# EnricoMiccoli/nodal

Measured on NVIDIA B200. Metric: unknowns_per_second, higher is better.
Workload: dtype f64

## Files before the change

__graft_entry__.py:

```python
import os
import subprocess
import sys

ROOT = os.path.dirname(os.path.abspath(__file__))
if ROOT not in sys.path:
    sys.path.insert(0, ROOT)


def build():
    subprocess.check_call(["make", "-C", os.path.join(ROOT, "nodal_b200", "csrc"), "-j8"])
    sys.path.insert(0, os.path.join(ROOT, "tests"))
    import helpers
    helpers.stamp_host_lib()
    helpers.amg_host_lib()
    import sources_host
    sources_host.sources_host_lib()
    import amg_cycle_host
    amg_cycle_host.amg_cycle_host_lib()
    ref_nodal = os.path.join(os.environ.get("NODAL_REFERENCE", "/root/reference"), "nodal")
    if os.path.isdir(ref_nodal) and not os.path.isfile(os.path.join(ROOT, "baseline", "_ref", "nodal", "nodal.py")):
        subprocess.call([sys.executable, os.path.join(ROOT, "baseline", "install_ref.py")])
    import nodal_b200
    from nodal_b200 import _lib
    _lib.load()


def smoke():
    import numpy as np
    import nodal_b200 as n
    import nodal_b200.equiv
    from nodal_b200 import dist as ndist
    from nodal_b200 import generators as gen
    from nodal_b200.device import Device
    from oracle import mna_oracle as orc

    N = 24
    r_cpu = orc.equivalent_resistance(orc.grid2d_rows(N), "1", "g", sparse=True, backend="dict")
    r_gpu = n.equiv.equivalent_resistance(gen.grid2d(N), "1", "g", sparse=True)
    r_jac = n.equiv.equivalent_resistance(gen.grid2d(N), "1", "g", sparse=True, precond="jacobi")
    r_amg = n.equiv.equivalent_resistance(gen.grid2d(N), "1", "g", sparse=True, precond="amg", amg={"coarse": 64})
    for r in (r_gpu, r_jac, r_amg):
        assert abs(r - r_cpu) <= 1e-9 * abs(r_cpu), (r, r_cpu)
    dev = Device.get(0)
    import copy
    net = copy.deepcopy(gen.grid2d(64))
    net.process_component(["a1", "A", "1", "1", "g"])
    table = net.table()
    csr, rhs = dev.assemble_csr(table)
    x, info = ndist.single_solver(dev).solve_amg(csr.n, np.array([0, csr.n], dtype=np.int32), csr.indptr, csr.indices,
                                                  csr.data, rhs, rtol=1e-10, gather_below=300)
    r_dist = float(x[net.nodenum["1"]])
    r64 = orc.equivalent_resistance(orc.grid2d_rows(64), "1", "g", sparse=True, backend="dict")
    assert info["status"] == 0 and info["distributed_levels"] >= 1 and abs(r_dist - r64) <= 1e-9 * abs(r64), (info, r_dist, r64)
    pg = gen.power_grid(16, 5, vdd=1.0, load=1e-3, seed=0)
    sol = n.Circuit(pg, sparse=True, eliminate_sources=True).solve()
    red = sol.stats["reduction"]
    assert red["eliminated"] and red["relres_full"] <= 1e-9 and np.all(sol.potentials() <= 1.0), sol.stats
    print(f"smoke ok: R({N}x{N} grid) default={float(r_gpu)!r} jacobi={float(r_jac)!r} amg={float(r_amg)!r} "
          f"oracle={float(r_cpu)!r}; R(64x64) partitioned-AMG form={r_dist!r} oracle={float(r64)!r}; "
          f"power grid 16x16 relres_full={red['relres_full']:.1e}")


if __name__ == "__main__":
    build()
    if len(sys.argv) > 1 and sys.argv[1] == "smoke":
        smoke()
```

include/nodal_b200.h:

```cpp
#ifndef NODAL_B200_H
#define NODAL_B200_H

#include <stdint.h>

#ifdef __cplusplus
extern "C" {
#endif

#define NODAL_ABI_VERSION 1

enum {
    NODAL_OK = 0,
    NODAL_SINGULAR = 1,
    NODAL_NOT_CONVERGED = 2,
    NODAL_BREAKDOWN = 3,
    NODAL_CUDA_ERROR = 4,
    NODAL_BAD_ARG = -1
};

enum { NODAL_T_R = 0, NODAL_T_A = 1, NODAL_T_E = 2, NODAL_T_VCVS = 3, NODAL_T_VCCS = 4,
       NODAL_T_CCVS = 5, NODAL_T_CCCS = 6 };
#define NODAL_GROUND (-1)
#define NODAL_UNUSED (-2)

typedef struct nodal_ctx nodal_ctx;

int nodal_abi_version(void);
const char* nodal_last_error(void);
uint64_t nodal_launch_count(void);
int nodal_ctx_create(int device, nodal_ctx** out);
int nodal_ctx_destroy(nodal_ctx* ctx);
int64_t nodal_ctx_workspace_bytes(nodal_ctx* ctx);

int nodal_stamp_coo(nodal_ctx* ctx, int64_t ncomp,
                    const uint8_t* type, const double* value,
                    const int32_t* a, const int32_t* b, const int32_t* c, const int32_t* d,
                    const int32_t* drv, const int32_t* branch,
                    int32_t kcl, int32_t n, int32_t stride, int32_t colbits,
                    uint64_t* keys, double* vals, void* stream);

int nodal_csr_build(nodal_ctx* ctx, int32_t n, int64_t nslots, int32_t colbits,
                    uint64_t* keys, double* vals, double* rhs,
                    int64_t* nnz_h, void* stream);
int nodal_csr_fetch(nodal_ctx* ctx, int32_t n, int64_t nnz,
                    int32_t* indptr, int32_t* indices, double* data, void* stream);
int nodal_csr_build_ordered(nodal_ctx* ctx, int32_t n, int64_t nslots, int32_t colbits,
                            uint64_t* keys, double* vals, int32_t order, double* rhs, int64_t* nnz_h,
                            void* stream);

int nodal_csr_to_dense(nodal_ctx* ctx, int32_t n, const int32_t* indptr, const int32_t* indices,
                       const double* data, double* G, void* stream);
int nodal_coo_to_dense_atomic(nodal_ctx* ctx, int32_t n, int64_t nslots, int32_t colbits,
                              const uint64_t* keys, const double* vals, double* G, double* rhs,
                              void* stream);

int nodal_spmv(nodal_ctx* ctx, int32_t n, int64_t nnz, const int32_t* indptr,
               const int32_t* indices, const double* data, const double* x, double* y,
               void* stream);

typedef struct nodal_sell nodal_sell;
int nodal_sell_create(nodal_ctx* ctx, int32_t n, int64_t nnz, const int32_t* indptr,
                      const int32_t* indices, const double* data, nodal_sell** out, void* stream);
int nodal_sell_destroy(nodal_sell* m);
int64_t nodal_sell_padded_nnz(const nodal_sell* m);
int nodal_sell_spmv(nodal_ctx* ctx, const nodal_sell* m, const double* x, double* y, void* stream);

int nodal_pcg(nodal_ctx* ctx, int32_t n, int64_t nnz, const int32_t* indptr,
              const int32_t* indices, const double* data, const double* rhs, double* x,
              double rtol, int32_t maxit, int32_t flags,
              int32_t* iters_h, double* relres_h, double* stats_h, void* stream);
#define NODAL_PCG_FORCE_CSR 1
#define NODAL_PCG_NO_GRAPH 2
#define NODAL_PCG_PROFILE 4
#define NODAL_PCG_NO_SCALE 8

int nodal_gmres(nodal_ctx* ctx, int32_t n, int64_t nnz, const int32_t* indptr,
                const int32_t* indices, const double* data, const double* rhs, double* x,
                double rtol, int32_t restart, int32_t maxit,
                int32_t* iters_h, double* relres_h, void* stream);

typedef struct nodal_amg nodal_amg;
int nodal_amg_create(nodal_ctx* ctx, int32_t n, int64_t nnz, const int32_t* indptr,
                     const int32_t* indices, const double* data, const double* params,
                     nodal_amg** out, void* stream);
int nodal_amg_destroy(nodal_amg* amg);
int nodal_amg_info(const nodal_amg* amg, int32_t cap, int32_t* nlevels, int64_t* rows, int64_t* nnz,
                   double* setup_ms, int32_t* direct);
int nodal_amg_fetch_level(nodal_ctx* ctx, const nodal_amg* amg, int32_t level, int32_t* agg,
                          int32_t* indptr, int32_t* indices, double* data, void* stream);
int nodal_amg_apply(nodal_ctx* ctx, const nodal_amg* amg, const double* r, double* z, void* stream);
int nodal_amg_pcg(nodal_ctx* ctx, nodal_amg* amg, const double* rhs, double* x, double rtol,
                  int32_t maxit, int32_t* iters_h, double* relres_h, double* stats_h, void* stream);

int nodal_connected_components(nodal_ctx* ctx, int64_t ncomp, const int32_t* a, const int32_t* b,
                               int32_t kcl, int32_t* labels, int32_t* ncomponents_h,
                               int32_t* reached_h, void* stream);

int nodal_source_forest(nodal_ctx* ctx, int64_t ncomp, const uint8_t* type, const double* value,
                        const int32_t* a, const int32_t* b, const int32_t* branch, int32_t kcl, int32_t be,
                        int32_t* erow, int32_t* adj_ptr, int32_t* adj_row, int32_t* rep_row, double* offset,
                        int32_t* parent_edge, int32_t* depth, int32_t* roots, int64_t* info_h, void* stream);
int nodal_source_reduce_scan(nodal_ctx* ctx, int64_t ncomp, const uint8_t* type, const int32_t* a,
                             const int32_t* b, int32_t kcl, const int32_t* rep_row, const double* offset,
                             uint32_t* pos, int64_t* count_h, void* stream);
int nodal_source_reduce_table(nodal_ctx* ctx, int64_t ncomp, const uint8_t* type, const double* value,
                              const int32_t* a, const int32_t* b, int32_t kcl, const int32_t* rep_row,
                              const double* offset, const uint32_t* pos, uint8_t* out_type, double* out_value,
                              int32_t* out_a, int32_t* out_b, void* stream);
int nodal_source_expand(nodal_ctx* ctx, int32_t kcl, int32_t n, int32_t nsrc, const int32_t* erow,
                        const int32_t* a, const int32_t* b, const int32_t* branch, const int32_t* adj_ptr,
                        const int32_t* adj_row, const int32_t* rep_row, const double* offset,
                        const int32_t* depth, int32_t max_depth, const double* y, const double* rhs,
                        int64_t nnz, const int32_t* indptr, const int32_t* indices, const double* data,
                        double* x, double* relres_h, void* stream);

int nodal_lu_solve(nodal_ctx* ctx, int32_t n, double* G, const double* rhs, double* x,
                   int32_t* info_h, void* stream);

int nodal_dgemm_sub_profile(nodal_ctx* ctx, double* C, const double* A, const double* B, int32_t M, int32_t N,
                            int32_t K, int32_t ld, int32_t reps, double* ms_out, void* stream);

int nodal_lu_batched(nodal_ctx* ctx, int64_t batch, int32_t ncomp,
                     const uint8_t* type, const int32_t* a, const int32_t* b,
                     const int32_t* c, const int32_t* d, const int32_t* drv, const int32_t* branch,
                     int32_t kcl, int32_t n, const double* values, double* x, int32_t* info,
                     void* stream);

int nodal_lu_batched_soa(nodal_ctx* ctx, int64_t batch, int32_t ncomp,
                         const uint8_t* type, const int32_t* a, const int32_t* b,
                         const int32_t* c, const int32_t* d, const int32_t* drv, const int32_t* branch,
                         int32_t kcl, int32_t n, const double* values_t, double* x_t, int32_t* info,
// ... 41 lines not shown
```

nodal_b200/_lib.py:

```python
from __future__ import annotations

import ctypes as C
import os

_HERE = os.path.dirname(os.path.abspath(__file__))
LIB_PATH = os.path.join(_HERE, "libnodal_b200.so")

OK, SINGULAR, NOT_CONVERGED, BREAKDOWN, CUDA_ERROR, BAD_ARG = 0, 1, 2, 3, 4, -1
PCG_FORCE_CSR, PCG_NO_GRAPH, PCG_PROFILE, PCG_NO_SCALE = 1, 2, 4, 8

_vp, _i32, _i64, _f64 = C.c_void_p, C.c_int32, C.c_int64, C.c_double

SIGNATURES = {
    "nodal_abi_version": (C.c_int, []),
    "nodal_last_error": (C.c_char_p, []),
    "nodal_launch_count": (C.c_uint64, []),
    "nodal_ctx_create": (C.c_int, [C.c_int, C.POINTER(_vp)]),
    "nodal_ctx_destroy": (C.c_int, [_vp]),
    "nodal_ctx_workspace_bytes": (_i64, [_vp]),
    "nodal_stamp_coo": (C.c_int, [_vp, _i64, _vp, _vp, _vp, _vp, _vp, _vp, _vp, _vp,
                                  _i32, _i32, _i32, _i32, _vp, _vp, _vp]),
    "nodal_csr_build": (C.c_int, [_vp, _i32, _i64, _i32, _vp, _vp, _vp, C.POINTER(_i64), _vp]),
    "nodal_csr_build_ordered": (C.c_int, [_vp, _i32, _i64, _i32, _vp, _vp, _i32, _vp, C.POINTER(_i64), _vp]),
    "nodal_csr_fetch": (C.c_int, [_vp, _i32, _i64, _vp, _vp, _vp, _vp]),
    "nodal_csr_to_dense": (C.c_int, [_vp, _i32, _vp, _vp, _vp, _vp, _vp]),
    "nodal_coo_to_dense_atomic": (C.c_int, [_vp, _i32, _i64, _i32, _vp, _vp, _vp, _vp, _vp]),
    "nodal_spmv": (C.c_int, [_vp, _i32, _i64, _vp, _vp, _vp, _vp, _vp, _vp]),
    "nodal_sell_create": (C.c_int, [_vp, _i32, _i64, _vp, _vp, _vp, C.POINTER(_vp), _vp]),
    "nodal_sell_destroy": (C.c_int, [_vp]),
    "nodal_sell_padded_nnz": (_i64, [_vp]),
    "nodal_sell_spmv": (C.c_int, [_vp, _vp, _vp, _vp, _vp]),
    "nodal_pcg": (C.c_int, [_vp, _i32, _i64, _vp, _vp, _vp, _vp, _vp, _f64, _i32, _i32,
                            C.POINTER(_i32), C.POINTER(_f64), C.POINTER(_f64), _vp]),
    "nodal_gmres": (C.c_int, [_vp, _i32, _i64, _vp, _vp, _vp, _vp, _vp, _f64, _i32, _i32,
                              C.POINTER(_i32), C.POINTER(_f64), _vp]),
    "nodal_amg_create": (C.c_int, [_vp, _i32, _i64, _vp, _vp, _vp, C.POINTER(_f64), C.POINTER(_vp), _vp]),
    "nodal_amg_destroy": (C.c_int, [_vp]),
    "nodal_amg_info": (C.c_int, [_vp, _i32, C.POINTER(_i32), C.POINTER(_i64), C.POINTER(_i64),
                                 C.POINTER(_f64), C.POINTER(_i32)]),
    "nodal_amg_fetch_level": (C.c_int, [_vp, _vp, _i32, _vp, _vp, _vp, _vp, _vp]),
    "nodal_amg_apply": (C.c_int, [_vp, _vp, _vp, _vp, _vp]),
    "nodal_amg_pcg": (C.c_int, [_vp, _vp, _vp, _vp, _f64, _i32, C.POINTER(_i32), C.POINTER(_f64),
                                C.POINTER(_f64), _vp]),
    "nodal_connected_components": (C.c_int, [_vp, _i64, _vp, _vp, _i32, _vp, C.POINTER(_i32),
                                             C.POINTER(_i32), _vp]),
    "nodal_source_forest": (C.c_int, [_vp, _i64, _vp, _vp, _vp, _vp, _vp, _i32, _i32] + [_vp] * 8
                            + [C.POINTER(_i64), _vp]),
    "nodal_source_reduce_scan": (C.c_int, [_vp, _i64, _vp, _vp, _vp, _i32, _vp, _vp, _vp, C.POINTER(_i64), _vp]),
    "nodal_source_reduce_table": (C.c_int, [_vp, _i64, _vp, _vp, _vp, _vp, _i32, _vp, _vp, _vp, _vp, _vp, _vp, _vp,
                                            _vp]),
    "nodal_source_expand": (C.c_int, [_vp, _i32, _i32, _i32] + [_vp] * 9 + [_i32, _vp, _vp, _i64, _vp, _vp, _vp, _vp,
                                                                             C.POINTER(_f64), _vp]),
    "nodal_lu_solve": (C.c_int, [_vp, _i32, _vp, _vp, _vp, C.POINTER(_i32), _vp]),
    "nodal_dgemm_sub_profile": (C.c_int, [_vp, _vp, _vp, _vp, _i32, _i32, _i32, _i32, _i32, C.POINTER(_f64), _vp]),
    "nodal_lu_batched": (C.c_int, [_vp, _i64, _i32, _vp, _vp, _vp, _vp, _vp, _vp, _vp,
                                   _i32, _i32, _vp, _vp, _vp, _vp]),
    "nodal_lu_batched_soa": (C.c_int, [_vp, _i64, _i32, _vp, _vp, _vp, _vp, _vp, _vp, _vp,
                                       _i32, _i32, _vp, _vp, _vp, _vp]),
    "nodal_dist_unique_id": (C.c_int, [_vp]),
    "nodal_dist_create": (C.c_int, [_vp, _vp, _i32, _i32, C.POINTER(_vp)]),
    "nodal_dist_create_single": (C.c_int, [_vp, C.POINTER(_vp)]),
    "nodal_dist_destroy": (C.c_int, [_vp]),
    "nodal_dist_pcg": (C.c_int, [_vp, _vp, _i32, _vp, _i64, _vp, _vp, _vp, _vp, _vp, _f64, _i32,
                                 C.POINTER(_i32), C.POINTER(_f64), C.POINTER(_f64), _vp]),
    "nodal_amg_pcg_multi": (C.c_int, [_vp, _vp, _i32, _vp, _vp, _f64, _i32, C.POINTER(_i32), C.POINTER(_f64),
                                      C.POINTER(_i32), _vp]),
    "nodal_amg_profile_sweeps": (C.c_int, [_vp, _vp, _i32, C.POINTER(_f64), _vp]),
    "nodal_amg_profile_cycle": (C.c_int, [_vp, _vp, _i32, C.POINTER(_f64), _vp]),
    "nodal_table_select_scan": (C.c_int, [_vp, _i64, _vp, _vp, _i32, _i32, _vp, C.POINTER(_i64), _vp]),
    "nodal_table_select_gather": (C.c_int, [_vp, _i64, _vp, _i32, _i32] + [_vp] * 16 + [_vp]),
    "nodal_dist_amg_pcg": (C.c_int, [_vp, _vp, _i32, _vp, _i64, _vp, _vp, _vp, _vp, _vp, C.POINTER(_f64), _f64,
                                     _i32, C.POINTER(_i32), C.POINTER(_f64), C.POINTER(_f64), _vp]),
}

_lib = None


class NodalLibraryError(RuntimeError):
    """The CUDA extension is missing or a CUDA call failed."""


def load():
    global _lib
    if _lib is not None:
        return _lib
    if not os.path.exists(LIB_PATH):
        raise NodalLibraryError(
            f"{LIB_PATH} not found: build it with `python -c 'import __graft_entry__ as g; g.build()'`"
            " (or `make -C nodal_b200/csrc`). nodal_b200 has no CPU fallback.")
    lib = C.CDLL(LIB_PATH)
    for name, (res, args) in SIGNATURES.items():
        fn = getattr(lib, name)
        fn.restype = res
        fn.argtypes = args
    if lib.nodal_abi_version() != 1:
        raise NodalLibraryError("libnodal_b200.so ABI version mismatch")
    _lib = lib
    return lib


def last_error():
    return load().nodal_last_error().decode("utf-8", "replace")


def check(status, what, allowed=(OK,)):
    if status in allowed:
        return status
# ... 2 lines not shown
```

nodal_b200/csrc/common.cuh:

```cuda
#pragma once
#include <cuda_runtime.h>
#include <stdint.h>
#include <stdio.h>
#include <string.h>
#include <string>
#include <vector>

#include "../../include/nodal_b200.h"

#include <nvtx3/nvToolsExt.h>

struct NvtxRange {
    explicit NvtxRange(const char* name) { nvtxRangePushA(name); }
    ~NvtxRange() { nvtxRangePop(); }
    NvtxRange(const NvtxRange&) = delete;
    NvtxRange& operator=(const NvtxRange&) = delete;
};

typedef unsigned long long u64;
typedef unsigned int u32;

#define NODAL_NUM_SMS_FALLBACK 148

void nodal_set_error(const char* fmt, ...);

#define CUDA_TRY(expr)                                                                   \
    do {                                                                                 \
        cudaError_t _e = (expr);                                                         \
        if (_e != cudaSuccess) {                                                         \
            nodal_set_error("%s:%d: %s -> %s", __FILE__, __LINE__, #expr,                \
                            cudaGetErrorString(_e));                                     \
            (void)cudaGetLastError();                       \
            return NODAL_CUDA_ERROR;                                                     \
        }                                                                                \
    } while (0)

#define NODAL_TRY(expr)                                                                  \
    do {                                                                                 \
        int _s = (expr);                                                                 \
        if (_s != NODAL_OK) return _s;                                                   \
    } while (0)

extern unsigned long long g_nodal_launches;
#define KERNEL_CHECK()                 \
    do {                               \
        ++g_nodal_launches;            \
        CUDA_TRY(cudaGetLastError());  \
    } while (0)

struct nodal_ctx {
    int device = 0;
    int num_sms = NODAL_NUM_SMS_FALLBACK;
    char* arena = nullptr;
    size_t arena_bytes = 0;
    size_t arena_used = 0;
    uint64_t generation = 0;
    void* pinned = nullptr;
    struct PoolBlock { void* ptr; size_t bytes; bool used; };
    std::vector<PoolBlock> pool;
};

void* ctx_pool_alloc(nodal_ctx* ctx, size_t bytes);
void ctx_pool_free(nodal_ctx* ctx, void* ptr);

int ctx_reserve(nodal_ctx* ctx, size_t bytes);
void* ctx_carve(nodal_ctx* ctx, size_t bytes);

template <typename T>
static inline T* carve(nodal_ctx* ctx, size_t count) {
    return reinterpret_cast<T*>(ctx_carve(ctx, count * sizeof(T)));
}
static inline size_t align_up(size_t x, size_t a) { return (x + a - 1) / a * a; }

#ifdef __CUDACC__
__device__ __forceinline__ double warp_sum(double v) {
#pragma unroll
    for (int o = 16; o > 0; o >>= 1) v += __shfl_xor_sync(0xffffffffu, v, o);
    return v;
}
__device__ __forceinline__ u32 lane_id() { return threadIdx.x & 31; }
__device__ __forceinline__ u32 lanemask_lt() {
    u32 m;
    asm("mov.u32 %0, %%lanemask_lt;" : "=r"(m));
    return m;
}

__device__ __forceinline__ double block_sum(double v, double* smem ) {
    v = warp_sum(v);
    const int w = threadIdx.x >> 5, nw = (blockDim.x + 31) >> 5;
    __syncthreads();
    if (lane_id() == 0) smem[w] = v;
    __syncthreads();
    if (w == 0) {
        double t = (lane_id() < nw) ? smem[lane_id()] : 0.0;
        t = warp_sum(t);
        if (lane_id() == 0) smem[32] = t;
    }
    __syncthreads();
    return smem[32];
}

__device__ __forceinline__ double reduce_partials(const double* __restrict__ part, int count,
                                                  double* smem) {
    double t = 0.0;
    for (int i = threadIdx.x; i < count; i += blockDim.x) t += part[i];
    return block_sum(t, smem);
}

__device__ __forceinline__ void reduce_partials3(const double* __restrict__ a, int na,
                                                 const double* __restrict__ b, int nb,
                                                 const double* __restrict__ c, int nc, double* smem,
                                                 double& sa, double& sb, double& sc) {
    double va[8], vb[8], vc[8];
#pragma unroll
    for (int k = 0; k < 8; ++k) {
        const int i = threadIdx.x + k * blockDim.x;
        va[k] = i < na ? a[i] : 0.0;
        vb[k] = i < nb ? b[i] : 0.0;
        vc[k] = i < nc ? c[i] : 0.0;
    }
    double ta = 0.0, tb = 0.0, tc = 0.0;
#pragma unroll
    for (int k = 0; k < 8; ++k) {
        const int i = threadIdx.x + k * blockDim.x;
        if (i < na) ta += va[k];
        if (i < nb) tb += vb[k];
        if (i < nc) tc += vc[k];
    }
    sa = block_sum(ta, smem);
    sb = nb > 0 ? block_sum(tb, smem) : 0.0;
    sc = nc > 0 ? block_sum(tc, smem) : 0.0;
}
#endif

int scan_exclusive_u32(nodal_ctx* ctx, const u32* in, u32* out, int64_t count, u32* total_dev,
                       cudaStream_t st);
size_t scan_scratch_bytes(int64_t count);
int radix_sort_pairs(nodal_ctx* ctx, u64* keys, u64* vals, u64* keys_alt, u64* vals_alt,
                     int64_t count, int bits, bool* result_in_alt, cudaStream_t st);
size_t radix_sort_scratch_bytes(int64_t count);
// ... 4 lines not shown
```

nodal_b200/csrc/csr.cu:

```cuda
#include "common.cuh"

constexpr int CB_THREADS = 256;

__global__ void __launch_bounds__(CB_THREADS)
mark_heads_kernel(const u64* __restrict__ keys, int64_t count, int32_t n, int colbits,
                  u32* __restrict__ head) {
    for (int64_t i = (int64_t)blockIdx.x * blockDim.x + threadIdx.x; i < count;
         i += (int64_t)gridDim.x * blockDim.x) {
        const u64 k = keys[i];
        const bool live = (int64_t)(k >> colbits) < (int64_t)n;
        head[i] = (live && (i == 0 || keys[i - 1] != k)) ? 1u : 0u;
    }
}

__global__ void __launch_bounds__(CB_THREADS)
segment_sum_kernel(const u64* __restrict__ keys, const double* __restrict__ vals, int64_t count,
                   int32_t n, int colbits, const u32* __restrict__ head_scan,
                   u64* __restrict__ ukey, double* __restrict__ uval, u32* __restrict__ keep,
                   double* __restrict__ rhs) {
    const u64 colmask = ((u64)1 << colbits) - 1;
    for (int64_t i = (int64_t)blockIdx.x * blockDim.x + threadIdx.x; i < count;
         i += (int64_t)gridDim.x * blockDim.x) {
        const u64 k = keys[i];
        if ((int64_t)(k >> colbits) >= (int64_t)n) continue;
        if (i != 0 && keys[i - 1] == k) continue;
        double s = vals[i];
        for (int64_t j = i + 1; j < count && keys[j] == k; ++j) s = s + vals[j];
        const u32 seg = head_scan[i];
        const int32_t col = (int32_t)(k & colmask);
        ukey[seg] = k;
        uval[seg] = s;
        if (col == n) {
            rhs[(int32_t)(k >> colbits)] = s;
            keep[seg] = 0u;
        } else {
            keep[seg] = (s != 0.0) ? 1u : 0u;
        }
    }
}

__global__ void __launch_bounds__(CB_THREADS)
iota_u64_kernel(int64_t count, u64* __restrict__ out) {
    for (int64_t i = (int64_t)blockIdx.x * blockDim.x + threadIdx.x; i < count; i += (int64_t)gridDim.x * blockDim.x)
        out[i] = (u64)i;
}

__global__ void __launch_bounds__(CB_THREADS)
segment_sum_first_touch_kernel(const u64* __restrict__ keys, const u64* __restrict__ idx, const double* __restrict__ vals,
                               int64_t count, int32_t n, int colbits, const u32* __restrict__ head_scan,
                               u64* __restrict__ ukey, double* __restrict__ uval, u32* __restrict__ keep,
                               u32* __restrict__ ufirst, double* __restrict__ rhs) {
    const u64 colmask = ((u64)1 << colbits) - 1;
    for (int64_t i = (int64_t)blockIdx.x * blockDim.x + threadIdx.x; i < count;
         i += (int64_t)gridDim.x * blockDim.x) {
        const u64 k = keys[i];
        if ((int64_t)(k >> colbits) >= (int64_t)n) continue;
        if (i != 0 && keys[i - 1] == k) continue;
        double s = 0.0;
        bool absent = true;
        u32 first = 0;
        for (int64_t j = i; j < count && keys[j] == k; ++j) {
            const double t = s + vals[idx[j]];
            if (t != 0.0) {
                if (absent) { first = (u32)idx[j]; absent = false; }
            } else {
                absent = true;
            }
            s = absent ? 0.0 : t;
        }
        const u32 seg = head_scan[i];
        const int32_t col = (int32_t)(k & colmask);
        ukey[seg] = k;
        uval[seg] = s;
        ufirst[seg] = first;
        if (col == n) {
            rhs[(int32_t)(k >> colbits)] = s;
            keep[seg] = 0u;
        } else {
            keep[seg] = absent ? 0u : 1u;
        }
    }
}

// ... 2 lines not shown
                        const u32* __restrict__ keep, int64_t useg, int colbits, u64* __restrict__ keys2,
                        u64* __restrict__ pos2) {
    for (int64_t s = (int64_t)blockIdx.x * blockDim.x + threadIdx.x; s < useg; s += (int64_t)gridDim.x * blockDim.x) {
        if (!keep[s]) continue;
        const u32 p = keep_scan[s];
        keys2[p] = ((ukey[s] >> colbits) << 32) | (u64)ufirst[s];
        pos2[p] = (u64)p;
    }
}

__global__ void __launch_bounds__(CB_THREADS)
permute_entries_kernel(int64_t nnz, const u64* __restrict__ pos, const int32_t* __restrict__ cols_in,
                       const double* __restrict__ vals_in, int32_t* __restrict__ cols_out, double* __restrict__ vals_out) {
    for (int64_t q = (int64_t)blockIdx.x * blockDim.x + threadIdx.x; q < nnz; q += (int64_t)gridDim.x * blockDim.x) {
        const u64 p = pos[q];
        cols_out[q] = cols_in[p];
        vals_out[q] = vals_in[p];
    }
}

__global__ void __launch_bounds__(CB_THREADS)
compact_kernel(const u64* __restrict__ ukey, const double* __restrict__ uval,
               const u32* __restrict__ keep_scan, const u32* __restrict__ keep_flag_src,
               int64_t useg, int colbits, int32_t* __restrict__ indices, double* __restrict__ data,
               int32_t* __restrict__ krow) {
    const u64 colmask = ((u64)1 << colbits) - 1;
    for (int64_t s = (int64_t)blockIdx.x * blockDim.x + threadIdx.x; s < useg;
         s += (int64_t)gridDim.x * blockDim.x) {
        if (!keep_flag_src[s]) continue;
        const u32 p = keep_scan[s];
        const u64 k = ukey[s];
        indices[p] = (int32_t)(k & colmask);
        data[p] = uval[s];
        krow[p] = (int32_t)(k >> colbits);
    }
}

struct RowGap { int32_t first, last, value; int32_t pad; };
constexpr int ROWPTR_INLINE = 32;
constexpr int ROWPTR_MAX_GAPS = 4096;

__device__ __forceinline__ void fill_rows(int32_t first, int32_t last, int32_t value,
                                          int32_t* __restrict__ indptr, RowGap* gaps, unsigned int* ngaps) {
    if (last - first < ROWPTR_INLINE) {
        for (int32_t q = first; q <= last; ++q) indptr[q] = value;
        return;
    }
    const unsigned int slot = atomicAdd(ngaps, 1u);
    if (slot < ROWPTR_MAX_GAPS) { gaps[slot].first = first; gaps[slot].last = last; gaps[slot].value = value; }
    else for (int32_t q = first; q <= last; ++q) indptr[q] = value;
}

__global__ void __launch_bounds__(CB_THREADS)
row_ptr_kernel(const int32_t* __restrict__ krow, int64_t nnz, int32_t n,
               int32_t* __restrict__ indptr, RowGap* gaps, unsigned int* ngaps) {
    for (int64_t p = (int64_t)blockIdx.x * blockDim.x + threadIdx.x; p < nnz;
         p += (int64_t)gridDim.x * blockDim.x) {
        const int32_t r = krow[p];
        const int32_t rp = p ? krow[p - 1] : -1;
        if (r != rp) fill_rows(rp + 1, r, (int32_t)p, indptr, gaps, ngaps);
        if (p == nnz - 1) fill_rows(r + 1, n, (int32_t)nnz, indptr, gaps, ngaps);
    }
}

__global__ void __launch_bounds__(CB_THREADS)
row_ptr_gaps_kernel(int32_t* __restrict__ indptr, const RowGap* __restrict__ gaps,
                    const unsigned int* __restrict__ ngaps) {
    const unsigned int count = min(*ngaps, (unsigned int)ROWPTR_MAX_GAPS);
    for (unsigned int g = 0; g < count; ++g) {
        const RowGap gp = gaps[g];
        for (int64_t q = (int64_t)gp.first + (int64_t)blockIdx.x * blockDim.x + threadIdx.x; q <= gp.last;
             q += (int64_t)gridDim.x * blockDim.x)
            indptr[q] = gp.value;
    }
}

static int grid_for(nodal_ctx* ctx, int64_t work, int threads) {
    int64_t b = (work + threads - 1) / threads;
    int64_t cap = (int64_t)ctx->num_sms * 16;
    if (b < 1) b = 1;
    return (int)(b < cap ? b : cap);
}

struct PendingCsr {
    nodal_ctx* ctx = nullptr;
    const u64* ukey = nullptr;
    const double* uval = nullptr;
    const u32* keep = nullptr;
    const u32* keep_scan = nullptr;
    int32_t* krow = nullptr;
    const u32* ufirst = nullptr;
    int order = 0;
    int64_t useg = 0, nnz = 0;
    int32_t n = 0;
    int colbits = 0;
    uint64_t generation = 0;
};
static thread_local PendingCsr g_pending;

static int csr_build_impl(nodal_ctx* ctx, int32_t n, int64_t nslots, int32_t colbits, uint64_t* keys_, double* vals,
                          double* rhs, int64_t* nnz_h, void* stream, int order);

extern "C" int nodal_csr_build(nodal_ctx* ctx, int32_t n, int64_t nslots, int32_t colbits,
                               uint64_t* keys_, double* vals, double* rhs, int64_t* nnz_h,
                               void* stream) {
    return csr_build_impl(ctx, n, nslots, colbits, keys_, vals, rhs, nnz_h, stream, 0);
}

extern "C" int nodal_csr_build_ordered(nodal_ctx* ctx, int32_t n, int64_t nslots, int32_t colbits,
                                       uint64_t* keys_, double* vals, int32_t order, double* rhs,
                                       int64_t* nnz_h, void* stream) {
    if (order != 0 && order != 1) return NODAL_BAD_ARG;
    return csr_build_impl(ctx, n, nslots, colbits, keys_, vals, rhs, nnz_h, stream, order);
}

static int csr_build_impl(nodal_ctx* ctx, int32_t n, int64_t nslots, int32_t colbits, uint64_t* keys_, double* vals,
                          double* rhs, int64_t* nnz_h, void* stream, int order) {
    NvtxRange nvtx_range("nodal_csr_build");
    if (!ctx || n < 0 || nslots < 0 || !nnz_h) return NODAL_BAD_ARG;
    if (nslots >= ((int64_t)1 << 31)) {
        nodal_set_error("nodal_csr_build: more than 2^31 triples are not supported");
        return NODAL_BAD_ARG;
    }
    cudaStream_t st = (cudaStream_t)stream;
    u64* keys = reinterpret_cast<u64*>(keys_);
    g_pending = PendingCsr();
    *nnz_h = 0;
    CUDA_TRY(cudaSetDevice(ctx->device));
    CUDA_TRY(cudaMemsetAsync(rhs, 0, sizeof(double) * (size_t)n, st));
    if (nslots == 0 || n == 0) {
        g_pending.ctx = ctx;
        g_pending.n = n;
        NODAL_TRY(ctx_reserve(ctx, 4096));
        g_pending.generation = ctx->generation;
        return NODAL_OK;
    }
    int rowbits = 1;
    while (((int64_t)n >> rowbits) != 0) ++rowbits;
    const int bits = colbits + rowbits;

    const size_t slots = (size_t)nslots;
    size_t need = 2 * align_up(slots * 8, 256) + 3 * align_up(slots * 4, 256) +
                  radix_sort_scratch_bytes(nslots) + 2 * scan_scratch_bytes(nslots) + (1 << 16);
    if (order == 1) need += 2 * align_up(slots * 8, 256) + align_up(slots * 4, 256);
    NODAL_TRY(ctx_reserve(ctx, need));
    u64* keys_alt = carve<u64>(ctx, slots);
    u64* vals_alt = carve<u64>(ctx, slots);
    u64* idx = order == 1 ? carve<u64>(ctx, slots) : nullptr;
    double* usum = order == 1 ? carve<double>(ctx, slots) : nullptr;
    u32* ufirst = order == 1 ? carve<u32>(ctx, slots) : nullptr;
    if (order == 1 && (!idx || !usum || !ufirst)) return NODAL_CUDA_ERROR;
    u32* head = carve<u32>(ctx, slots);
    u32* keep = carve<u32>(ctx, slots);
    u32* keep_scan = carve<u32>(ctx, slots);
    u32* totals = carve<u32>(ctx, 64);
    if (!keys_alt || !vals_alt || !head || !keep || !keep_scan || !totals) return NODAL_CUDA_ERROR;

    bool in_alt = false;
    const size_t mark = ctx->arena_used;
    const int grid = grid_for(ctx, nslots, CB_THREADS);
    if (order == 1) {
        iota_u64_kernel<<<grid, CB_THREADS, 0, st>>>(nslots, idx);
        KERNEL_CHECK();
    }
    NODAL_TRY(radix_sort_pairs(ctx, keys, order == 1 ? idx : reinterpret_cast<u64*>(vals), keys_alt, vals_alt, nslots,
                               bits, &in_alt, st));
    ctx->arena_used = mark;
    const u64* sk = in_alt ? keys_alt : keys;
    const double* sv = in_alt ? reinterpret_cast<double*>(vals_alt) : vals;
    const u64* sidx = in_alt ? vals_alt : idx;
    u64* ukey = in_alt ? keys : keys_alt;
    double* uval = order == 1 ? usum : (in_alt ? vals : reinterpret_cast<double*>(vals_alt));

    mark_heads_kernel<<<grid, CB_THREADS, 0, st>>>(sk, nslots, n, colbits, head);
    KERNEL_CHECK();
    NODAL_TRY(scan_exclusive_u32(ctx, head, head, nslots, totals + 0, st));
    ctx->arena_used = mark;
    if (order == 1)
        segment_sum_first_touch_kernel<<<grid, CB_THREADS, 0, st>>>(sk, sidx, vals, nslots, n, colbits, head, ukey, uval,
                                                                    keep, ufirst, rhs);
    else
        segment_sum_kernel<<<grid, CB_THREADS, 0, st>>>(sk, sv, nslots, n, colbits, head, ukey, uval, keep, rhs);
    KERNEL_CHECK();
    u32* host_tot = reinterpret_cast<u32*>(ctx->pinned);
    CUDA_TRY(cudaMemcpyAsync(host_tot, totals, sizeof(u32), cudaMemcpyDeviceToHost, st));
    CUDA_TRY(cudaStreamSynchronize(st));
    NODAL_TRY(radix_sort_check(ctx));
    const int64_t useg = host_tot[0];
    NODAL_TRY(scan_exclusive_u32(ctx, keep, keep_scan, useg, totals + 1, st));
    CUDA_TRY(cudaMemcpyAsync(host_tot + 1, totals + 1, sizeof(u32), cudaMemcpyDeviceToHost, st));
    CUDA_TRY(cudaStreamSynchronize(st));
    const int64_t nnz = host_tot[1];

    g_pending.ctx = ctx;
    g_pending.ukey = ukey;
    g_pending.uval = uval;
    g_pending.keep = keep;
    g_pending.keep_scan = keep_scan;
    g_pending.krow = reinterpret_cast<int32_t*>(head);
    g_pending.ufirst = ufirst;
    g_pending.order = order;
    g_pending.useg = useg;
    g_pending.nnz = nnz;
    g_pending.n = n;
    g_pending.colbits = colbits;
    g_pending.generation = ctx->generation;
    *nnz_h = nnz;
    return NODAL_OK;
}

extern "C" int nodal_csr_fetch(nodal_ctx* ctx, int32_t n, int64_t nnz, int32_t* indptr,
                               int32_t* indices, double* data, void* stream) {
    PendingCsr& p = g_pending;
    if (!ctx || p.ctx != ctx || p.n != n || p.nnz != nnz ||
        ctx->generation != p.generation) {
        nodal_set_error("nodal_csr_fetch: no matching nodal_csr_build result is pending on this ctx");
        return NODAL_BAD_ARG;
    }
    cudaStream_t st = (cudaStream_t)stream;
    CUDA_TRY(cudaSetDevice(ctx->device));
    if (nnz == 0) {
        CUDA_TRY(cudaMemsetAsync(indptr, 0, sizeof(int32_t) * ((size_t)n + 1), st));
        g_pending = PendingCsr();
        return NODAL_OK;
    }
    compact_kernel<<<grid_for(ctx, p.useg, CB_THREADS), CB_THREADS, 0, st>>>(
        p.ukey, p.uval, p.keep_scan, p.keep, p.useg, p.colbits, indices, data, p.krow);
    KERNEL_CHECK();
    RowGap* gaps = reinterpret_cast<RowGap*>(ctx_pool_alloc(ctx, sizeof(RowGap) * ROWPTR_MAX_GAPS + 256));
    if (!gaps) return NODAL_CUDA_ERROR;
    unsigned int* ngaps = reinterpret_cast<unsigned int*>(gaps + ROWPTR_MAX_GAPS);
    CUDA_TRY(cudaMemsetAsync(ngaps, 0, sizeof(unsigned int), st));
    row_ptr_kernel<<<grid_for(ctx, nnz, CB_THREADS), CB_THREADS, 0, st>>>(p.krow, nnz, n, indptr, gaps, ngaps);
    KERNEL_CHECK();
    row_ptr_gaps_kernel<<<ctx->num_sms * 4, CB_THREADS, 0, st>>>(indptr, gaps, ngaps);
    KERNEL_CHECK();
    ctx_pool_free(ctx, gaps);
    if (p.order == 1 && nnz > 1) {
        int rowbits = 1;
        while (((int64_t)n >> rowbits) != 0) ++rowbits;
        const size_t cnt = (size_t)nnz;
        u64* k2 = static_cast<u64*>(ctx_pool_alloc(ctx, cnt * 8));
        u64* p2 = static_cast<u64*>(ctx_pool_alloc(ctx, cnt * 8));
        u64* k2a = static_cast<u64*>(ctx_pool_alloc(ctx, cnt * 8));
        u64* p2a = static_cast<u64*>(ctx_pool_alloc(ctx, cnt * 8));
        int32_t* ctmp = static_cast<int32_t*>(ctx_pool_alloc(ctx, cnt * 4));
        double* vtmp = static_cast<double*>(ctx_pool_alloc(ctx, cnt * 8));
        char* sort_ws = static_cast<char*>(ctx_pool_alloc(ctx, radix_sort_scratch_bytes(nnz) + 4096));
        int rc = (k2 && p2 && k2a && p2a && ctmp && vtmp && sort_ws) ? NODAL_OK : NODAL_CUDA_ERROR;
        if (rc == NODAL_OK) {
            first_touch_keys_kernel<<<grid_for(ctx, p.useg, CB_THREADS), CB_THREADS, 0, st>>>(
                p.ukey, p.ufirst, p.keep_scan, p.keep, p.useg, p.colbits, k2, p2);
            ++g_nodal_launches;
            char* arena = ctx->arena; const size_t bytes = ctx->arena_bytes, used = ctx->arena_used;
            ctx->arena = sort_ws; ctx->arena_bytes = radix_sort_scratch_bytes(nnz) + 4096; ctx->arena_used = 0;
            bool in_alt = false;
            rc = radix_sort_pairs(ctx, k2, p2, k2a, p2a, nnz, 32 + rowbits, &in_alt, st);
            ctx->arena = arena; ctx->arena_bytes = bytes; ctx->arena_used = used;
            if (rc == NODAL_OK) {
                cudaMemcpyAsync(ctmp, indices, cnt * 4, cudaMemcpyDeviceToDevice, st);
                cudaMemcpyAsync(vtmp, data, cnt * 8, cudaMemcpyDeviceToDevice, st);
                permute_entries_kernel<<<grid_for(ctx, nnz, CB_THREADS), CB_THREADS, 0, st>>>(
                    nnz, in_alt ? p2a : p2, ctmp, vtmp, indices, data);
                ++g_nodal_launches;
                if (cudaGetLastError() != cudaSuccess) rc = NODAL_CUDA_ERROR;
            }
        }
        for (void* q : {(void*)k2, (void*)p2, (void*)k2a, (void*)p2a, (void*)ctmp, (void*)vtmp, (void*)sort_ws})
            ctx_pool_free(ctx, q);
        if (rc != NODAL_OK) { g_pending = PendingCsr(); return rc; }
    }
    g_pending = PendingCsr();
    return NODAL_OK;
}

__global__ void __launch_bounds__(CB_THREADS)
csr_to_dense_kernel(int32_t n, const int32_t* __restrict__ indptr,
                    const int32_t* __restrict__ indices, const double* __restrict__ data,
                    double* __restrict__ G) {
    const int lane = threadIdx.x & 31;
    const int64_t warp = ((int64_t)blockIdx.x * blockDim.x + threadIdx.x) >> 5;
    const int64_t nwarps = ((int64_t)gridDim.x * blockDim.x) >> 5;
    for (int64_t r = warp; r < n; r += nwarps) {
        const int32_t e = indptr[r + 1];
        for (int32_t j = indptr[r] + lane; j < e; j += 32)
            G[(size_t)r * n + indices[j]] = data[j];
    }
}

extern "C" int nodal_csr_to_dense(nodal_ctx* ctx, int32_t n, const int32_t* indptr,
                                  const int32_t* indices, const double* data, double* G,
                                  void* stream) {
    if (!ctx || n < 0) return NODAL_BAD_ARG;
    if (n == 0) return NODAL_OK;
    cudaStream_t st = (cudaStream_t)stream;
    CUDA_TRY(cudaSetDevice(ctx->device));
    CUDA_TRY(cudaMemsetAsync(G, 0, sizeof(double) * (size_t)n * n, st));
    csr_to_dense_kernel<<<grid_for(ctx, (int64_t)n * 32, CB_THREADS), CB_THREADS, 0, st>>>(
        n, indptr, indices, data, G);
    KERNEL_CHECK();
    return NODAL_OK;
}

__global__ void __launch_bounds__(CB_THREADS)
coo_to_dense_atomic_kernel(int32_t n, int64_t nslots, int colbits, const u64* __restrict__ keys,
// ... 53 lines not shown
```

Measured before the change: 144.1 million.

## Build CSR via per-row counting buckets instead of global radix sort

Replaces the default unordered CSR build with a counting-sort bucket scheme. Triples are counted and placed per row, then each row is sorted and reduced by a thread, warp or CTA tier chosen by row length. This avoids the full 64-bit radix sort of all triples. It adds an extra host sync to detect rows too long for the bucket path, which then fall back to the sort path. Warp-aggregated atomics keep the count and place steps cheap.

```diff
diff --git a/__graft_entry__.py b/__graft_entry__.py
--- a/__graft_entry__.py
+++ b/__graft_entry__.py
@@ -17,6 +17,8 @@
     sources_host.sources_host_lib()
     import amg_cycle_host
     amg_cycle_host.amg_cycle_host_lib()
+    import csr_host
+    csr_host.csr_host_lib()
     ref_nodal = os.path.join(os.environ.get("NODAL_REFERENCE", "/root/reference"), "nodal")
     if os.path.isdir(ref_nodal) and not os.path.isfile(os.path.join(ROOT, "baseline", "_ref", "nodal", "nodal.py")):
         subprocess.call([sys.executable, os.path.join(ROOT, "baseline", "install_ref.py")])
diff --git a/include/nodal_b200.h b/include/nodal_b200.h
--- a/include/nodal_b200.h
+++ b/include/nodal_b200.h
@@ -39,6 +39,7 @@
                     int32_t kcl, int32_t n, int32_t stride, int32_t colbits,
                     uint64_t* keys, double* vals, void* stream);
 
+#define NODAL_CSR_BUCKET_MAX_ROW 4096
 int nodal_csr_build(nodal_ctx* ctx, int32_t n, int64_t nslots, int32_t colbits,
                     uint64_t* keys, double* vals, double* rhs,
                     int64_t* nnz_h, void* stream);
@@ -47,6 +48,7 @@
 int nodal_csr_build_ordered(nodal_ctx* ctx, int32_t n, int64_t nslots, int32_t colbits,
                             uint64_t* keys, double* vals, int32_t order, double* rhs, int64_t* nnz_h,
                             void* stream);
+int nodal_csr_set_builder(nodal_ctx* ctx, int32_t builder);
 
 int nodal_csr_to_dense(nodal_ctx* ctx, int32_t n, const int32_t* indptr, const int32_t* indices,
                        const double* data, double* G, void* stream);
diff --git a/nodal_b200/_lib.py b/nodal_b200/_lib.py
--- a/nodal_b200/_lib.py
+++ b/nodal_b200/_lib.py
@@ -23,6 +23,7 @@
     "nodal_csr_build": (C.c_int, [_vp, _i32, _i64, _i32, _vp, _vp, _vp, C.POINTER(_i64), _vp]),
     "nodal_csr_build_ordered": (C.c_int, [_vp, _i32, _i64, _i32, _vp, _vp, _i32, _vp, C.POINTER(_i64), _vp]),
     "nodal_csr_fetch": (C.c_int, [_vp, _i32, _i64, _vp, _vp, _vp, _vp]),
+    "nodal_csr_set_builder": (C.c_int, [_vp, _i32]),
     "nodal_csr_to_dense": (C.c_int, [_vp, _i32, _vp, _vp, _vp, _vp, _vp]),
     "nodal_coo_to_dense_atomic": (C.c_int, [_vp, _i32, _i64, _i32, _vp, _vp, _vp, _vp, _vp]),
     "nodal_spmv": (C.c_int, [_vp, _i32, _i64, _vp, _vp, _vp, _vp, _vp, _vp]),
diff --git a/nodal_b200/csrc/common.cuh b/nodal_b200/csrc/common.cuh
--- a/nodal_b200/csrc/common.cuh
+++ b/nodal_b200/csrc/common.cuh
@@ -56,6 +56,7 @@
     size_t arena_used = 0;
     uint64_t generation = 0;
     void* pinned = nullptr;
+    int csr_builder = -1;
     struct PoolBlock { void* ptr; size_t bytes; bool used; };
     std::vector<PoolBlock> pool;
 };
diff --git a/nodal_b200/csrc/csr.cu b/nodal_b200/csrc/csr.cu
--- a/nodal_b200/csrc/csr.cu
+++ b/nodal_b200/csrc/csr.cu
@@ -1,4 +1,9 @@
+#include <stdlib.h>
+
+#include <algorithm>
+
 #include "common.cuh"
+#include "csr_core.cuh"
 
 constexpr int CB_THREADS = 256;
 
@@ -167,8 +172,276 @@
     return (int)(b < cap ? b : cap);
 }
 
+struct __align__(16) BucketSlot {
+    u64 key;
+    double val;
+};
+constexpr int BK_SHORT_THREADS = 128;
+constexpr int BK_SHORT_MAX = 16;
+constexpr int BK_WARP_THREADS = 256;
+constexpr int BK_WARP_MAX = 32;
+constexpr int BK_LONG_THREADS = 512;
+constexpr int BK_LONG_MAX = NODAL_CSR_BUCKET_MAX_ROW;
+static_assert((BK_LONG_MAX & (BK_LONG_MAX - 1)) == 0, "the CTA tier sorts a power of two");
+
+__device__ __forceinline__ u32 bucket_peers(int32_t row) {
+    return __match_any_sync(0xffffffffu, row >= 0 ? (u32)row : (0x80000000u | lane_id()));
+}
+
+__global__ void __launch_bounds__(CB_THREADS)
+bucket_count_kernel(const u64* __restrict__ keys, int64_t count, int32_t n, int colbits, u32* __restrict__ cnt,
+                    u32* __restrict__ too_long) {
+    const int64_t stride = (int64_t)gridDim.x * blockDim.x;
+    const int64_t rounds = (count + stride - 1) / stride;
+    for (int64_t it = 0; it < rounds; ++it) {
+        const int64_t i = it * stride + (int64_t)blockIdx.x * blockDim.x + threadIdx.x;
+        const int32_t row = i < count ? csr_live_row(keys[i], colbits, n) : -1;
+        const u32 peers = bucket_peers(row);
+        if (row >= 0 && (peers & lanemask_lt()) == 0u) {
+            const u32 m = (u32)__popc(peers);
+            if (atomicAdd(&cnt[row], m) + m > (u32)BK_LONG_MAX) *too_long = 1u;
+        }
+    }
+}
+
+__global__ void __launch_bounds__(CB_THREADS)
+bucket_place_kernel(const u64* __restrict__ keys, const double* __restrict__ vals, int64_t count, int32_t n,
+                    int colbits, u32* __restrict__ cur, BucketSlot* __restrict__ bs) {
+    const u64 colmask = ((u64)1 << colbits) - 1;
+    const int64_t stride = (int64_t)gridDim.x * blockDim.x;
+    const int64_t rounds = (count + stride - 1) / stride;
+    for (int64_t it = 0; it < rounds; ++it) {
+        const int64_t i = it * stride + (int64_t)blockIdx.x * blockDim.x + threadIdx.x;
+        u64 k = 0;
+        int32_t row = -1;
+        if (i < count) {
+            k = keys[i];
+            row = csr_live_row(k, colbits, n);
+        }
+        const u32 peers = bucket_peers(row);
+        const int leader = __ffs(peers) - 1;
+        u32 base = 0;
+        if (row >= 0 && (int)lane_id() == leader) base = atomicAdd(&cur[row], (u32)__popc(peers));
+        base = __shfl_sync(0xffffffffu, base, leader);
+        if (row >= 0) {
+            const u32 slot = base + (u32)__popc(peers & lanemask_lt());
+            bs[slot] = BucketSlot{csr_entry_key((int32_t)(k & colmask), (u32)i), vals[i]};
+        }
+    }
+}
+
+__global__ void __launch_bounds__(BK_SHORT_THREADS)
+bucket_rows_short_kernel(int32_t n, const u32* __restrict__ off, const u32* __restrict__ cnt, BucketSlot* __restrict__ bs, u32* __restrict__ kcnt, double* __restrict__ rhs,
+                         u32* __restrict__ warp_rows, u32* __restrict__ nwarp, u32* __restrict__ long_rows,
+                         u32* __restrict__ nlong) {
+    __shared__ u64 s_key[BK_SHORT_MAX * BK_SHORT_THREADS];
+    __shared__ double s_val[BK_SHORT_MAX * BK_SHORT_THREADS];
+    auto key = [&](int i) -> u64& { return s_key[i * BK_SHORT_THREADS + threadIdx.x]; };
+    auto val = [&](int i) -> double& { return s_val[i * BK_SHORT_THREADS + threadIdx.x]; };
+    for (int32_t r = blockIdx.x * blockDim.x + threadIdx.x; r < n; r += gridDim.x * blockDim.x) {
+        const int len = (int)cnt[r];
+        if (len > BK_WARP_MAX) {
+            long_rows[atomicAdd(nlong, 1u)] = (u32)r;
+            continue;
+        }
+        if (len > BK_SHORT_MAX) {
+            warp_rows[atomicAdd(nwarp, 1u)] = (u32)r;
+            continue;
+        }
+        const u32 o = off[r];
+        for (int j = 0; j < len; ++j) {
+            const BucketSlot e = bs[o + j];
+            key(j) = e.key;
+            val(j) = e.val;
+        }
+        for (int j = 1; j < len; ++j) csr_insert(key, val, j, key(j), val(j));
+        const int kept = csr_reduce_row(key, val, len, n, &rhs[r]);
+        for (int j = 0; j < kept; ++j) {
+            bs[o + j] = BucketSlot{key(j), val(j)};
+        }
+        kcnt[r] = (u32)kept;
+    }
+}
+
+__global__ void __launch_bounds__(BK_WARP_THREADS)
+bucket_rows_warp_kernel(int32_t n, const u32* __restrict__ off, const u32* __restrict__ cnt,
+                        const u32* __restrict__ warp_rows, const u32* __restrict__ nwarp, BucketSlot* __restrict__ bs, u32* __restrict__ kcnt, double* __restrict__ rhs) {
+    constexpr int WPB = BK_WARP_THREADS / 32;
+    __shared__ u64 s_key[WPB][BK_WARP_MAX];
+    __shared__ double s_val[WPB][BK_WARP_MAX];
+    const int w = threadIdx.x >> 5, lane = lane_id();
+    auto key = [&](int i) -> u64& { return s_key[w][i]; };
+    auto val = [&](int i) -> double& { return s_val[w][i]; };
+    const u32 count = *nwarp;
+    for (u32 q = blockIdx.x * WPB + w; q < count; q += gridDim.x * WPB) {
+        const u32 r = warp_rows[q];
+        const int len = (int)cnt[r];
+        const u32 o = off[r];
+        u64 k = ~0ull;
+        double v = 0.0;
+        if (lane < len) {
+            const BucketSlot e = bs[o + lane];
+            k = e.key;
+            v = e.val;
+        }
+        int rank = 0;
+        for (int j = 0; j < len; ++j) rank += __shfl_sync(0xffffffffu, k, j) < k ? 1 : 0;
+        if (lane < len) {
+            key(rank) = k;
+            val(rank) = v;
+        }
+        __syncwarp();
+        bool keep = false;
+        int32_t c = 0;
+        double s = 0.0;
+        if (lane < len) {
+            c = csr_entry_col(key(lane));
+            if (lane == 0 || csr_entry_col(key(lane - 1)) != c) {
+                csr_run_sum(key, val, lane, len, s);
+                if (c == n) rhs[r] = s;
+                keep = csr_keep(c, s, n);
+            }
+        }
+        const u32 kept = __ballot_sync(0xffffffffu, keep);
+        if (keep) {
+            const u32 pos = o + (u32)__popc(kept & lanemask_lt());
+            bs[pos] = BucketSlot{(u64)(u32)c, s};
+        }
+        if (lane == 0) kcnt[r] = (u32)__popc(kept);
+        __syncwarp();
+    }
+}
+
+__device__ __forceinline__ u32 block_exclusive_scan(u32 v, u32* s_warp ) {
+    const int lane = lane_id(), w = threadIdx.x >> 5, nw = (blockDim.x + 31) >> 5;
+    u32 x = v;
+#pragma unroll
+    for (int d = 1; d < 32; d <<= 1) {
+        const u32 y = __shfl_up_sync(0xffffffffu, x, d);
+        if (lane >= d) x += y;
+    }
+    if (lane == 31) s_warp[w] = x;
+    __syncthreads();
+    if (w == 0) {
+        const u32 t = lane < nw ? s_warp[lane] : 0u;
+        u32 z = t;
+#pragma unroll
+        for (int d = 1; d < 32; d <<= 1) {
+            const u32 y = __shfl_up_sync(0xffffffffu, z, d);
+            if (lane >= d) z += y;
+        }
+        if (lane < nw) s_warp[lane] = z - t;
+        if (lane == 31) s_warp[32] = z;
+    }
+    __syncthreads();
+    return s_warp[w] + x - v;
+}
+
+__global__ void __launch_bounds__(BK_LONG_THREADS)
+bucket_rows_long_kernel(int32_t n, const u32* __restrict__ off, const u32* __restrict__ cnt,
+                        const u32* __restrict__ long_rows, const u32* __restrict__ nlong, BucketSlot* __restrict__ bs, u32* __restrict__ kcnt, double* __restrict__ rhs) {
+    extern __shared__ u64 s_dyn[];
+    u64* s_key = s_dyn;
+    double* s_val = reinterpret_cast<double*>(s_dyn + BK_LONG_MAX);
+    __shared__ u32 s_scan[33];
+    auto key = [&](int i) -> u64& { return s_key[i]; };
+    auto val = [&](int i) -> double& { return s_val[i]; };
+    const u32 count = *nlong;
+    for (u32 q = blockIdx.x; q < count; q += gridDim.x) {
+        const u32 r = long_rows[q];
+        const int len = (int)cnt[r];
+        const u32 o = off[r];
+        int p2 = 1;
+        while (p2 < len) p2 <<= 1;
+        for (int i = threadIdx.x; i < p2; i += blockDim.x) {
+            if (i < len) {
+                const BucketSlot e = bs[o + i];
+                s_key[i] = e.key;
+                s_val[i] = e.val;
+            } else {
+                s_key[i] = ~0ull;
+            }
+        }
+        __syncthreads();
+        for (int k = 2; k <= p2; k <<= 1) {
+            for (int j = k >> 1; j > 0; j >>= 1) {
+                for (int i = threadIdx.x; i < p2; i += blockDim.x) {
+                    const int ixj = i ^ j;
+                    if (ixj > i) {
+                        const u64 a = s_key[i], b = s_key[ixj];
+                        if ((a > b) == ((i & k) == 0)) {
+                            s_key[i] = b; s_key[ixj] = a;
+                            const double t = s_val[i]; s_val[i] = s_val[ixj]; s_val[ixj] = t;
+                        }
+                    }
+                }
+                __syncthreads();
+            }
+        }
+        const int chunk = (len + (int)blockDim.x - 1) / (int)blockDim.x;
+        const int lo = min(len, (int)threadIdx.x * chunk), hi = min(len, lo + chunk);
+        u32 mine = 0;
+        for (int i = lo; i < hi; ++i) {
+            if (i > 0 && csr_entry_col(s_key[i]) == csr_entry_col(s_key[i - 1])) continue;
+            double s;
+            csr_run_sum(key, val, i, len, s);
+            mine += csr_keep(csr_entry_col(s_key[i]), s, n) ? 1u : 0u;
+        }
+        u32 pos = o + block_exclusive_scan(mine, s_scan);
+        for (int i = lo; i < hi; ++i) {
+            if (i > 0 && csr_entry_col(s_key[i]) == csr_entry_col(s_key[i - 1])) continue;
+            const int32_t c = csr_entry_col(s_key[i]);
+            double s;
+            csr_run_sum(key, val, i, len, s);
+            if (c == n) rhs[r] = s;
+            else if (csr_keep(c, s, n)) {
+                bs[pos] = BucketSlot{(u64)(u32)c, s};
+                ++pos;
+            }
+        }
+        if (threadIdx.x == 0) kcnt[r] = s_scan[32];
+        __syncthreads();
+    }
+}
+
+__global__ void __launch_bounds__(CB_THREADS)
+bucket_compact_kernel(int32_t n, const u32* __restrict__ off, const u32* __restrict__ kcnt,
+                      const u32* __restrict__ rowptr, const BucketSlot* __restrict__ bs,
+                      int32_t* __restrict__ indptr, int32_t* __restrict__ indices, double* __restrict__ data) {
+    for (int32_t r = blockIdx.x * blockDim.x + threadIdx.x; r < n; r += gridDim.x * blockDim.x) {
+        const u32 o = off[r], k = kcnt[r], p = rowptr[r];
+        for (u32 j = 0; j < k; ++j) {
+            const BucketSlot e = bs[o + j];
+            indices[p + j] = (int32_t)e.key;
+            data[p + j] = e.val;
+        }
+        indptr[r] = (int32_t)p;
+        if (r == n - 1) indptr[n] = (int32_t)(p + k);
+    }
+}
+
+static bool use_buckets(const nodal_ctx* ctx) {
+    if (ctx->csr_builder >= 0) return ctx->csr_builder == 0;
+    static const bool sort = [] {
+        const char* e = getenv("NODAL_CSR_SORT");
+        return e && *e && strcmp(e, "0") != 0;
+    }();
+    return !sort;
+}
+
+extern "C" int nodal_csr_set_builder(nodal_ctx* ctx, int32_t builder) {
+    if (!ctx || builder < -1 || builder > 1) return NODAL_BAD_ARG;
+    ctx->csr_builder = builder;
+    return NODAL_OK;
+}
+
 struct PendingCsr {
     nodal_ctx* ctx = nullptr;
+    bool buckets = false;
+    const u32* b_off = nullptr;
+    const u32* b_kcnt = nullptr;
+    const u32* b_rowptr = nullptr;
+    const BucketSlot* b_slot = nullptr;
     const u64* ukey = nullptr;
     const double* uval = nullptr;
     const u32* keep = nullptr;
@@ -199,6 +472,74 @@
     return csr_build_impl(ctx, n, nslots, colbits, keys_, vals, rhs, nnz_h, stream, order);
 }
 
+static int bucket_build(nodal_ctx* ctx, int32_t n, int64_t nslots, int32_t colbits, const u64* keys,
+                        const double* vals, double* rhs, int64_t* nnz_h, cudaStream_t st, bool* fallback) {
+    NvtxRange nvtx_range("csr_bucket_build");
+    *fallback = false;
+    const size_t rows = (size_t)n, slots = (size_t)nslots;
+    const size_t warp_cap = std::min<size_t>(rows, slots / (BK_SHORT_MAX + 1) + 1);
+    const size_t long_cap = std::min<size_t>(rows, slots / (BK_WARP_MAX + 1) + 1);
+    const size_t need = 4 * align_up(rows * 4, 256) + align_up(warp_cap * 4, 256) + align_up(long_cap * 4, 256) +
+                        2 * align_up(slots * 8, 256) + scan_scratch_bytes(n) + (1 << 16);
+    NODAL_TRY(ctx_reserve(ctx, need));
+    u32* cnt = carve<u32>(ctx, rows);
+    u32* off = carve<u32>(ctx, rows);
+    u32* cur = carve<u32>(ctx, rows);
+    u32* rowptr = carve<u32>(ctx, rows);
+    u32* warp_rows = carve<u32>(ctx, warp_cap);
+    u32* long_rows = carve<u32>(ctx, long_cap);
+    BucketSlot* bs = carve<BucketSlot>(ctx, slots);
+    u32* totals = carve<u32>(ctx, 64);
+    if (!cnt || !off || !cur || !rowptr || !warp_rows || !long_rows || !bs || !totals) return NODAL_CUDA_ERROR;
+    const size_t mark = ctx->arena_used;
+    CUDA_TRY(cudaMemsetAsync(cnt, 0, rows * 4, st));
+    CUDA_TRY(cudaMemsetAsync(totals, 0, 64 * 4, st));
+    const int grid = grid_for(ctx, nslots, CB_THREADS);
+    bucket_count_kernel<<<grid, CB_THREADS, 0, st>>>(keys, nslots, n, colbits, cnt, totals + 1);
+    KERNEL_CHECK();
+    u32* host_tot = reinterpret_cast<u32*>(ctx->pinned);
+    CUDA_TRY(cudaMemcpyAsync(host_tot + 1, totals + 1, sizeof(u32), cudaMemcpyDeviceToHost, st));
+    CUDA_TRY(cudaStreamSynchronize(st));
+    if (host_tot[1]) {
+        *fallback = true;
+        return NODAL_OK;
+    }
+    NODAL_TRY(scan_exclusive_u32(ctx, cnt, off, n, totals + 3, st));
+    ctx->arena_used = mark;
+    CUDA_TRY(cudaMemcpyAsync(cur, off, rows * 4, cudaMemcpyDeviceToDevice, st));
+    bucket_place_kernel<<<grid, CB_THREADS, 0, st>>>(keys, vals, nslots, n, colbits, cur, bs);
+    KERNEL_CHECK();
+    u32* kcnt = cur;
+    bucket_rows_short_kernel<<<grid_for(ctx, n, BK_SHORT_THREADS), BK_SHORT_THREADS, 0, st>>>(
+        n, off, cnt, bs, kcnt, rhs, warp_rows, totals + 4, long_rows, totals + 2);
+    KERNEL_CHECK();
+    bucket_rows_warp_kernel<<<ctx->num_sms * 8, BK_WARP_THREADS, 0, st>>>(n, off, cnt, warp_rows, totals + 4, bs,
+                                                                          kcnt, rhs);
+    KERNEL_CHECK();
+    const int dyn = 2 * BK_LONG_MAX * (int)sizeof(u64);
+    CUDA_TRY(cudaFuncSetAttribute(bucket_rows_long_kernel, cudaFuncAttributeMaxDynamicSharedMemorySize, dyn));
+    bucket_rows_long_kernel<<<ctx->num_sms * 2, BK_LONG_THREADS, dyn, st>>>(n, off, cnt, long_rows, totals + 2, bs,
+                                                                            kcnt, rhs);
+    KERNEL_CHECK();
+    NODAL_TRY(scan_exclusive_u32(ctx, kcnt, rowptr, n, totals + 0, st));
+    ctx->arena_used = mark;
+    CUDA_TRY(cudaMemcpyAsync(host_tot, totals, sizeof(u32), cudaMemcpyDeviceToHost, st));
+    CUDA_TRY(cudaStreamSynchronize(st));
+    const int64_t nnz = host_tot[0];
+    g_pending.ctx = ctx;
+    g_pending.buckets = true;
+    g_pending.b_off = off;
+    g_pending.b_kcnt = kcnt;
+    g_pending.b_rowptr = rowptr;
+    g_pending.b_slot = bs;
+    g_pending.nnz = nnz;
+    g_pending.n = n;
+    g_pending.colbits = colbits;
+    g_pending.generation = ctx->generation;
+    *nnz_h = nnz;
+    return NODAL_OK;
+}
+
 static int csr_build_impl(nodal_ctx* ctx, int32_t n, int64_t nslots, int32_t colbits, uint64_t* keys_, double* vals,
                           double* rhs, int64_t* nnz_h, void* stream, int order) {
     NvtxRange nvtx_range("nodal_csr_build");
@@ -219,6 +560,12 @@
         NODAL_TRY(ctx_reserve(ctx, 4096));
         g_pending.generation = ctx->generation;
         return NODAL_OK;
+    }
+    if (order == 0 && use_buckets(ctx)) {
+        bool fallback = false;
+        NODAL_TRY(bucket_build(ctx, n, nslots, colbits, keys, vals, rhs, nnz_h, st, &fallback));
+        if (!fallback) return NODAL_OK;
+        g_pending = PendingCsr();
     }
     int rowbits = 1;
     while (((int64_t)n >> rowbits) != 0) ++rowbits;
@@ -306,6 +653,13 @@
     CUDA_TRY(cudaSetDevice(ctx->device));
     if (nnz == 0) {
         CUDA_TRY(cudaMemsetAsync(indptr, 0, sizeof(int32_t) * ((size_t)n + 1), st));
+        g_pending = PendingCsr();
+        return NODAL_OK;
+    }
+    if (p.buckets) {
+        bucket_compact_kernel<<<grid_for(ctx, n, CB_THREADS), CB_THREADS, 0, st>>>(
+            n, p.b_off, p.b_kcnt, p.b_rowptr, p.b_slot, indptr, indices, data);
+        KERNEL_CHECK();
         g_pending = PendingCsr();
         return NODAL_OK;
     }
diff --git a/nodal_b200/csrc/csr_core.cuh b/nodal_b200/csrc/csr_core.cuh
--- /dev/null
+++ b/nodal_b200/csrc/csr_core.cuh
@@ -0,0 +1,60 @@
+#pragma once
+#include <stdint.h>
+
+#ifndef __CUDACC__
+#define __host__
+#define __device__
+#endif
+
+__host__ __device__ inline int32_t csr_live_row(unsigned long long key, int colbits, int32_t n) {
+    const unsigned long long r = key >> colbits;
+    return r < (unsigned long long)(uint32_t)n ? (int32_t)r : -1;
+}
+
+__host__ __device__ inline unsigned long long csr_entry_key(int32_t col, uint32_t emission) {
+    return ((unsigned long long)(uint32_t)col << 32) | (unsigned long long)emission;
+}
+__host__ __device__ inline int32_t csr_entry_col(unsigned long long k) { return (int32_t)(k >> 32); }
+
+template <typename Keys, typename Vals>
+__host__ __device__ inline void csr_insert(Keys key, Vals val, int j, unsigned long long k, double v) {
+    int i = j;
+    while (i > 0 && key(i - 1) > k) {
+        key(i) = key(i - 1);
+        val(i) = val(i - 1);
+        --i;
+    }
+    key(i) = k;
+    val(i) = v;
+}
+
+template <typename Keys, typename Vals>
+__host__ __device__ inline int csr_run_sum(Keys key, Vals val, int i, int len, double& s) {
+    const int32_t c = csr_entry_col(key(i));
+    s = val(i);
+    int j = i + 1;
+    while (j < len && csr_entry_col(key(j)) == c) {
+        s = s + val(j);
+        ++j;
+    }
+    return j;
+}
+
+__host__ __device__ inline bool csr_keep(int32_t c, double s, int32_t n) { return c != n && s != 0.0; }
+
+template <typename Keys, typename Vals>
+__host__ __device__ inline int csr_reduce_row(Keys key, Vals val, int len, int32_t n, double* rhs) {
+    int kept = 0;
+    for (int i = 0; i < len;) {
+        const int32_t c = csr_entry_col(key(i));
+        double s;
+        i = csr_run_sum(key, val, i, len, s);
+        if (c == n) *rhs = s;
+        else if (csr_keep(c, s, n)) {
+            key(kept) = (unsigned long long)(uint32_t)c;
+            val(kept) = s;
+            ++kept;
+        }
+    }
+    return kept;
+}
```

New measurement: 154.2 million, median of 6. +7.0%, better.
